# fugue-project/fugue

Hardware: NVIDIA H100
Metric: transform() rows/sec, hash-partitioned (num=256) identity map, 8-col table (higher is better)
Workload: dtype int64+f64 (byte moves; u64 hash arithmetic)

## Files before the change

### fugue_b200/csrc/fb_partition.cu

```cuda
#include <stdlib.h>

#include <mutex>

#include "fb_common.cuh"

namespace {

constexpr int kBlock = 512;
constexpr int kItems = 8;
constexpr int kTile = kBlock * kItems;
constexpr int kWarps = kBlock / 32;
constexpr int kCtasPerSm = 2;

struct FbCols {
  const void* src[FB_MAX_COLS];
  void* dst[FB_MAX_COLS];
  int32_t width[FB_MAX_COLS];
  int32_t ncols;
};

struct ChunkGeom {
  int64_t nrows;
  int64_t full_rows;
  int64_t tiles_per_chunk;
// ... 172 lines not shown
    const uint4 c = ((const uint4*)my)[lane];
    ((uint4*)(rec + kMetaCnt))[lane] = c;
    acc[0] += c.x & 0xFFFFu; acc[1] += c.x >> 16;
    acc[2] += c.y & 0xFFFFu; acc[3] += c.y >> 16;
    acc[4] += c.z & 0xFFFFu; acc[5] += c.z >> 16;
    acc[6] += c.w & 0xFFFFu; acc[7] += c.w >> 16;
    ((uint4*)my)[lane] = make_uint4(0, 0, 0, 0);
    __syncwarp();
  }
#pragma unroll
  for (int i = 0; i < 8; ++i)
    if (acc[i] != 0) atomicAdd(&s_hist[lane * 8 + i], acc[i]);
  __syncthreads();
  if (threadIdx.x < num) hist[(size_t)blockIdx.x * num + threadIdx.x] = s_hist[threadIdx.x];
}

__global__ void __launch_bounds__(256)
fb_scan_chunks_kernel(uint32_t* __restrict__ hist, uint32_t num, int32_t nchunks,
                      int64_t* __restrict__ totals) {
  __shared__ uint32_t s_warp[8];
  __shared__ uint32_t s_carry;
  const uint32_t b = blockIdx.x;
  const unsigned lane = threadIdx.x & 31, warp = threadIdx.x >> 5;
  if (threadIdx.x == 0) s_carry = 0;
  __syncthreads();
  for (int32_t c0 = 0; c0 < nchunks; c0 += 256) {
    int32_t c = c0 + threadIdx.x;
    uint32_t v = c < nchunks ? hist[(size_t)c * num + b] : 0;
    uint32_t x = v;
#pragma unroll
    for (int o = 1; o < 32; o <<= 1) {
      uint32_t y = __shfl_up_sync(0xFFFFFFFFu, x, o);
      if (lane >= (unsigned)o) x += y;
    }
    if (lane == 31) s_warp[warp] = x;
    __syncthreads();
    uint32_t wbase = 0;
    for (unsigned w = 0; w < warp; ++w) wbase += s_warp[w];
    uint32_t carry = s_carry;
    if (c < nchunks) hist[(size_t)c * num + b] = carry + wbase + x - v;
    __syncthreads();
    if (threadIdx.x == 255) s_carry = carry + wbase + x;
    __syncthreads();
  }
  if (threadIdx.x == 0) totals[b] = (int64_t)s_carry;
}

__global__ void __launch_bounds__(1024)
fb_scan_parts_kernel(int64_t* __restrict__ offsets, uint32_t num) {
  __shared__ int64_t s_warp[32];
  __shared__ int64_t s_carry;
  const unsigned lane = threadIdx.x & 31, warp = threadIdx.x >> 5;
  if (threadIdx.x == 0) s_carry = 0;
  __syncthreads();
  for (uint32_t b0 = 0; b0 < num; b0 += 1024) {
    uint32_t b = b0 + threadIdx.x;
    int64_t v = b < num ? offsets[b] : 0;
    int64_t x = v;
#pragma unroll
    for (int o = 1; o < 32; o <<= 1) {
      int64_t y = __shfl_up_sync(0xFFFFFFFFu, x, o);
      if (lane >= (unsigned)o) x += y;
    }
    if (lane == 31) s_warp[warp] = x;
    __syncthreads();
    int64_t wbase = 0;
    for (unsigned w = 0; w < warp; ++w) wbase += s_warp[w];
    int64_t carry = s_carry;
    if (b < num) offsets[b] = carry + wbase + x - v;
    __syncthreads();
    if (threadIdx.x == 1023) s_carry = carry + wbase + x;
    __syncthreads();
  }
  if (threadIdx.x == 0) offsets[num] = s_carry;
}

__host__ __device__ inline uint32_t nb_padded(uint32_t num) { return (num + 1 + 3) & ~3u; }

__host__ __device__ inline size_t scatter_smem_bytes(uint32_t num) {
  size_t nbp = nb_padded(num);
  return 2 * (size_t)kTile * 8 + (3 + (size_t)kWarps) * nbp * 4 + 32 * 4 + (size_t)kTile * 2;
}

constexpr int kMaxPer = (FB_MAX_PARTITIONS + 1 + kBlock - 1) / kBlock;

struct TileCtx {
  uint64_t* buf;
  uint32_t* delta;
  uint32_t* cursor;
  uint32_t* bin_start;
  uint32_t* cnt;
  uint32_t* scanw;
  uint16_t* pid_sorted;
  uint32_t nbp;
};

template <typename T, bool kFull>
__device__ __forceinline__ void load_col(const void* __restrict__ src, int64_t warp_row0, int warp_rows,
                                         unsigned lane, T (&v)[kItems]) {
  const T* __restrict__ p = (const T*)src + warp_row0 + lane;
#pragma unroll
  for (int r = 0; r < kItems; ++r)
    if (kFull || r * 32 + (int)lane < warp_rows) v[r] = __ldg(p + r * 32);
}

template <typename T, bool kFull>
__device__ __forceinline__ void move_columns(const FbCols& cols, const TileCtx& cx,
                                             const uint32_t (&pos)[kItems], const uint32_t (&dst)[kItems],
                                             int64_t warp_row0, int warp_rows, int tile_rows,
                                             unsigned lane, int& phase) {
  int c = 0;
  while (c < cols.ncols && cols.width[c] != (int)sizeof(T)) ++c;
  if (c >= cols.ncols) return;
  T v[kItems];
  load_col<T, kFull>(cols.src[c], warp_row0, warp_rows, lane, v);
  while (c < cols.ncols) {
    T* __restrict__ buf = (T*)(cx.buf + (size_t)(phase & 1) * kTile);
#pragma unroll
    for (int r = 0; r < kItems; ++r) buf[pos[r]] = v[r];
    int nxt = c + 1;
    while (nxt < cols.ncols && cols.width[nxt] != (int)sizeof(T)) ++nxt;
    if (nxt < cols.ncols) load_col<T, kFull>(cols.src[nxt], warp_row0, warp_rows, lane, v);
    __syncthreads();
    T* __restrict__ out = (T*)cols.dst[c];
#pragma unroll
    for (int k = 0; k < kItems; ++k) {
      const int j = k * kBlock + (int)threadIdx.x;
      if (kFull || j < tile_rows) out[dst[k]] = buf[j];
    }
    ++phase;
    c = nxt;
  }
}

template <bool kSingleU64, int kBits, bool kFull, bool kAll8>
__device__ __forceinline__ void scatter_tile(const FbKeys& keys, const FbDiv& dv, const uint32_t num,
                                             const FbCols& cols, const TileCtx& cx,
                                             const int64_t tile_row0, const int tile_rows, int& phase) {
  const unsigned lane = threadIdx.x & 31, warp = threadIdx.x >> 5;
  const unsigned lt = fb_lanemask_lt();
  const uint32_t nb = num + 1;
  const uint32_t nbp = cx.nbp;
  uint32_t* __restrict__ my_cnt = cx.cnt + warp * nbp;
  const int64_t warp_row0 = tile_row0 + (int64_t)warp * (32 * kItems);
  const int warp_rows = tile_rows - (int)warp * (32 * kItems);

  uint32_t pid[kItems];
#pragma unroll
  for (int r = 0; r < kItems; ++r) {
    const bool ok = kFull || (r * 32 + (int)lane) < warp_rows;
    pid[r] = ok ? compute_pid<kSingleU64>(keys, dv, warp_row0 + r * 32 + lane) : num;
  }

  uint32_t pos[kItems];
#pragma unroll
  for (int r = 0; r < kItems; ++r) {
    const unsigned m = match_lanes<kBits + (kFull ? 0 : 1)>(pid[r], 0xFFFFFFFFu);
    const unsigned before = __popc(m & lt);
    uint32_t old = 0;
    if (before == 0) {
      old = my_cnt[pid[r]];
      my_cnt[pid[r]] = old + __popc(m);
    }
    __syncwarp();
    old = __shfl_sync(0xFFFFFFFFu, old, __ffs(m) - 1);
    pos[r] = old + before;
  }
  __syncthreads();

  {
    const uint32_t per = (nb + kBlock - 1) / kBlock;
    const uint32_t b0 = threadIdx.x * per;
    uint32_t tot[kMaxPer];
    uint32_t sum = 0;
#pragma unroll
    for (int i = 0; i < kMaxPer; ++i) {
      tot[i] = 0;
      if ((uint32_t)i < per && b0 + i < nb) {
        uint32_t run = 0;
#pragma unroll
        for (int w = 0; w < kWarps; ++w) {
          const uint32_t t = cx.cnt[w * nbp + b0 + i];
          cx.cnt[w * nbp + b0 + i] = run;
          run += t;
        }
        tot[i] = run;
        sum += run;
      }
    }
    uint32_t x = sum;
#pragma unroll
    for (int o = 1; o < 32; o <<= 1) {
      const uint32_t y = __shfl_up_sync(0xFFFFFFFFu, x, o);
      if (lane >= (unsigned)o) x += y;
    }
    if (lane == 31) cx.scanw[warp] = x;
    __syncthreads();
    uint32_t run = x - sum;
    {
      const uint32_t wt = lane < kWarps ? cx.scanw[lane] : 0;
#pragma unroll
      for (int w = 0; w < kWarps; ++w) {
        const uint32_t v = __shfl_sync(0xFFFFFFFFu, wt, w);
        if ((unsigned)w < warp) run += v;
      }
    }
#pragma unroll
    for (int i = 0; i < kMaxPer; ++i) {
      if ((uint32_t)i < per && b0 + i < nb) {
        const uint32_t cur = cx.cursor[b0 + i];
        cx.bin_start[b0 + i] = run;
        cx.delta[b0 + i] = cur - run;
        cx.cursor[b0 + i] = cur + tot[i];
        run += tot[i];
      }
    }
  }
  __syncthreads();

#pragma unroll
  for (int r = 0; r < kItems; ++r) {
    pos[r] += cx.bin_start[pid[r]] + my_cnt[pid[r]];
    cx.pid_sorted[pos[r]] = (uint16_t)pid[r];
  }
  __syncthreads();
  uint32_t dst[kItems];
#pragma unroll
  for (int k = 0; k < kItems; ++k) {
    const int j = k * kBlock + (int)threadIdx.x;
    dst[k] = cx.delta[cx.pid_sorted[j]] + (uint32_t)j;
  }
  for (uint32_t i = threadIdx.x; i < (uint32_t)kWarps * nbp; i += kBlock) cx.cnt[i] = 0;

  move_columns<uint64_t, kFull>(cols, cx, pos, dst, warp_row0, warp_rows, tile_rows, lane, phase);
  if (!kAll8) {
    move_columns<uint32_t, kFull>(cols, cx, pos, dst, warp_row0, warp_rows, tile_rows, lane, phase);
    move_columns<uint16_t, kFull>(cols, cx, pos, dst, warp_row0, warp_rows, tile_rows, lane, phase);
    move_columns<uint8_t, kFull>(cols, cx, pos, dst, warp_row0, warp_rows, tile_rows, lane, phase);
  }
  __syncthreads();
}

template <bool kSingleU64, int kBits, bool kAll8>
__global__ void __launch_bounds__(kBlock, kCtasPerSm)
fb_scatter_kernel(FbKeys keys, FbDiv dv, uint32_t num, ChunkGeom g, int chunk0,
                  const uint32_t* __restrict__ chunk_base, const int64_t* __restrict__ part_offsets,
                  FbCols cols) {
  extern __shared__ __align__(128) uint64_t smem64[];
  TileCtx cx;
  cx.nbp = nb_padded(num);
  cx.buf = smem64;
  cx.delta = (uint32_t*)(smem64 + 2 * kTile);
  cx.cursor = cx.delta + cx.nbp;
  cx.bin_start = cx.cursor + cx.nbp;
  cx.cnt = cx.bin_start + cx.nbp;
  cx.scanw = cx.cnt + kWarps * cx.nbp;
  cx.pid_sorted = (uint16_t*)(cx.scanw + 32);

  const int chunk = chunk0 + (int)blockIdx.x;
  int64_t chunk_row0, chunk_row1;
  chunk_range(g, chunk, chunk_row0, chunk_row1);

  for (uint32_t b = threadIdx.x; b < cx.nbp; b += kBlock)
    cx.cursor[b] = b < num ? (uint32_t)part_offsets[b] + chunk_base[(size_t)chunk * num + b] : 0u;
  for (uint32_t i = threadIdx.x; i < (uint32_t)kWarps * cx.nbp; i += kBlock) cx.cnt[i] = 0;
  __syncthreads();

  int phase = 0;
  for (int64_t tile_row0 = chunk_row0; tile_row0 < chunk_row1; tile_row0 += kTile) {
    const int64_t left = chunk_row1 - tile_row0;
    if (left >= kTile)
      scatter_tile<kSingleU64, kBits, true, kAll8>(keys, dv, num, cols, cx, tile_row0, kTile, phase);
    else
      scatter_tile<kSingleU64, kBits, false, kAll8>(keys, dv, num, cols, cx, tile_row0, (int)left, phase);
  }
}

constexpr int kSwcMaxCols = 8;
constexpr uint32_t kSwcMaxNum = 256;

__device__ __forceinline__ uint32_t smem_u32(const void* p) { return (uint32_t)__cvta_generic_to_shared(p); }

__device__ __forceinline__ void mbar_init(uint32_t bar, uint32_t count) {
  asm volatile("mbarrier.init.shared::cta.b64 [%0], %1;" ::"r"(bar), "r"(count) : "memory");
}
__device__ __forceinline__ void mbar_expect_tx(uint32_t bar, uint32_t bytes) {
  asm volatile("mbarrier.arrive.expect_tx.shared::cta.b64 _, [%0], %1;" ::"r"(bar), "r"(bytes) : "memory");
}
__device__ __forceinline__ void mbar_arrive_relaxed(uint32_t bar) {
  asm volatile("mbarrier.arrive.relaxed.cta.shared::cta.b64 _, [%0];" ::"r"(bar) : "memory");
}
__device__ __forceinline__ void mbar_wait(uint32_t bar, uint32_t parity) {
  asm volatile(
      "{\n"
      ".reg .pred p;\n"
      "FB_WAIT:\n"
      "mbarrier.try_wait.parity.shared::cta.b64 p, [%0], %1;\n"
      "@p bra FB_DONE;\n"
      "bra FB_WAIT;\n"
      "FB_DONE:\n"
      "}\n" ::"r"(bar), "r"(parity)
      : "memory");
}
__device__ __forceinline__ uint64_t l2_policy_evict_first() {
  uint64_t pol;
  asm volatile("createpolicy.fractional.L2::evict_first.b64 %0, 1.0;" : "=l"(pol));
  return pol;
}
__device__ __forceinline__ uint64_t l2_policy_evict_last() {
  uint64_t pol;
  asm volatile("createpolicy.fractional.L2::evict_last.b64 %0, 1.0;" : "=l"(pol));
  return pol;
}
__device__ __forceinline__ void tma_load_1d(uint32_t dst_smem, const void* src, uint32_t bytes, uint32_t bar,
                                            uint64_t policy) {
  asm volatile(
      "cp.async.bulk.shared::cluster.global.mbarrier::complete_tx::bytes.L2::cache_hint [%0], [%1], %2, [%3], %4;"
      ::"r"(dst_smem), "l"(src), "r"(bytes), "r"(bar), "l"(policy)
      : "memory");
}

constexpr int kWsMoverWarps = 16, kWsRankWarps = 8;
constexpr int kWsMovers = kWsMoverWarps * 32, kWsRankers = kWsRankWarps * 32;
constexpr int kWsThreads = kWsMovers + kWsRankers + 128;
constexpr int kWsG = 16;
constexpr int kWsGWide = 4;
constexpr int kWsMinStages = 3;
constexpr int kWsRankItems = 16;
constexpr uint32_t kWsProducerRegs = 24, kWsRankerRegs = 64, kWsMoverRegs = 88;
static_assert(128 * kWsProducerRegs + kWsRankers * kWsRankerRegs + kWsMovers * kWsMoverRegs <= kWsThreads * 72,
              "setmaxnreg: the roles take more registers than the launch gives the CTA");
constexpr int kMoveBatch = 8;

struct WsUnits {
  const uint64_t* src[FB_MAX_COLS];
  uint64_t* dst[FB_MAX_COLS];
  int32_t nunits;
  int32_t per_group;
  int32_t ngroups;
};

struct WsMap {
  const uint64_t* src2[FB_MAX_COLS];
  uint64_t a[FB_MAX_COLS], b[FB_MAX_COLS], c[FB_MAX_COLS];
  int32_t mode[FB_MAX_COLS];
};

__device__ __forceinline__ uint64_t ws_apply_map(int mode, bool two, uint64_t x, uint64_t y, uint64_t a, uint64_t b,
                                                 uint64_t c) {
  if (mode == 1) {
    double r = __dmul_rn(__longlong_as_double((long long)a), __longlong_as_double((long long)x));
    if (two) r = __dadd_rn(r, __dmul_rn(__longlong_as_double((long long)b), __longlong_as_double((long long)y)));
    return (uint64_t)__double_as_longlong(__dadd_rn(r, __longlong_as_double((long long)c)));
  }
  if (mode == 2) return a * x + (two ? b * y : 0ULL) + c;
  return x;
}

template <int G, int RI>
__host__ __device__ inline size_t ws_book_bytes(uint32_t num, int ncols) {
  constexpr size_t kT = (size_t)kWsRankers * RI;
  const size_t nbp = nb_padded(num);
  const size_t E = (size_t)num * (G - 1);
  size_t b = 64 * 8;
  b += (size_t)ncols * E * 8;
  b += (kT + E) * 4;
  b += 5 * nbp * 4 + 64 * 4;
  b += ((E * 2 + 15) / 16) * 16;
  b += 2 * (size_t)kMetaBytes + 128;
  return b;
}

__device__ __forceinline__ void mbar_arrive(uint32_t bar) {
  asm volatile("mbarrier.arrive.shared::cta.b64 _, [%0];" ::"r"(bar) : "memory");
}
__device__ __forceinline__ void mover_sync() { asm volatile("bar.sync 1, %0;" ::"n"(kWsMovers) : "memory"); }
__device__ __forceinline__ void ranker_sync() { asm volatile("bar.sync 2, %0;" ::"n"(kWsRankers) : "memory"); }
template <uint32_t N>
__device__ __forceinline__ void setmaxnreg_dec() { asm volatile("setmaxnreg.dec.sync.aligned.u32 %0;" ::"n"(N)); }
template <uint32_t N>
__device__ __forceinline__ void setmaxnreg_inc() { asm volatile("setmaxnreg.inc.sync.aligned.u32 %0;" ::"n"(N)); }

template <int kBits, int G, int kWsRankItems, bool kMap>
__global__ void __launch_bounds__(kWsThreads, 1)
fb_scatter_ws_kernel(WsUnits units, uint32_t num, ChunkGeom g, int nstages,
                     const uint8_t* __restrict__ meta,
                     const uint32_t* __restrict__ chunk_base, const int64_t* __restrict__ part_offsets,
                     const __grid_constant__ WsMap map) {
  constexpr uint32_t T = (uint32_t)kWsRankers * kWsRankItems;
  static_assert(T == (uint32_t)kTile, "pass 1 ranks tiles of kTile rows");
  static_assert(G >= 2 && G <= 16 && (G & (G - 1)) == 0, "G must be a power of two <= 16");
  constexpr uint32_t GM = G - 1;
  constexpr uint32_t kStageBytes = T * 8;
  constexpr int kSlotRounds = ((int)T + (int)kSwcMaxNum * (G - 1) + kWsMovers - 1) / kWsMovers;
  constexpr int kEntryRoundsM = ((int)kSwcMaxNum * (G - 1) + kWsMovers - 1) / kWsMovers;
  extern __shared__ __align__(128) uint64_t smem64[];
  const uint32_t nbp = nb_padded(num);
  const uint32_t E = num * GM;
  const int grp = (int)blockIdx.x % units.ngroups;
  const int chunk_first = (int)blockIdx.x / units.ngroups, chunk_step = (int)gridDim.x / units.ngroups;
  const int u0 = grp * units.per_group;
  const int ncols = min(units.per_group, units.nunits - u0);
  uint64_t* ring = smem64;
  uint64_t* bars = ring + (size_t)nstages * T;
  uint64_t* carry = bars + 64;
  uint32_t* slotinfo = (uint32_t*)(carry + (size_t)ncols * E);
  uint32_t* wpos = slotinfo + T + E;
  uint32_t* kcnt = wpos + nbp;
  uint32_t* binfo = kcnt + nbp;
  uint32_t* wstart = binfo + nbp;
  uint32_t* wdelta = wstart + nbp;
  uint32_t* scanw = wdelta + nbp;
  uint16_t* carryinfo = (uint16_t*)(scanw + 64);
  uint8_t* metabuf = (uint8_t*)(((uintptr_t)(carryinfo + E) + 127) & ~(uintptr_t)127);

  const unsigned lane = threadIdx.x & 31, warp = threadIdx.x >> 5;
  const uint32_t bar_full = smem_u32(bars), bar_empty = smem_u32(bars + 16);
  const uint32_t bar_pid_full = smem_u32(bars + 32), bar_pid_empty = smem_u32(bars + 34);
  const uint32_t bar_slots_ready = smem_u32(bars + 36), bar_slots_free = smem_u32(bars + 37);
  const uint32_t bar_flush_done = smem_u32(bars + 38);

  if (threadIdx.x == 0) {
    for (int s = 0; s < nstages; ++s) {
      mbar_init(bar_full + 8 * s, 1);
      mbar_init(bar_empty + 8 * s, kWsMoverWarps);
    }
    for (int i = 0; i < 2; ++i) {
      mbar_init(bar_pid_full + 8 * i, 1);
      mbar_init(bar_pid_empty + 8 * i, kWsRankWarps);
    }
    mbar_init(bar_slots_ready, kWsRankWarps);
    mbar_init(bar_slots_free, kWsMoverWarps);
    mbar_init(bar_flush_done, kWsMoverWarps);
    asm volatile("fence.mbarrier_init.release.cluster;" ::: "memory");
  }
  __syncthreads();

  if (warp >= kWsMoverWarps + kWsRankWarps) {
    setmaxnreg_dec<kWsProducerRegs>();
    if (warp == kWsMoverWarps + kWsRankWarps && lane == 0) {
      const uint64_t pol = l2_policy_evict_first(), meta_pol = l2_policy_evict_last();
      const uint32_t ring_s = smem_u32(ring), meta_s = smem_u32(metabuf);
      uint32_t s = 0, ph = 0, seq = 0;
      int chunk = chunk_first;
      int64_t r0 = 0, r1 = 0, t0 = 0;
      bool have = chunk < g.nchunks_full;
      if (have) { chunk_range(g, chunk, r0, r1); t0 = r0; }
      auto load_pid = [&](int64_t row0, uint32_t q) {
        const uint32_t b = q & 1, pp = (q >> 1) & 1;
        mbar_wait(bar_pid_empty + 8 * b, pp ^ 1);
        mbar_expect_tx(bar_pid_full + 8 * b, kMetaBytes);
        tma_load_1d(meta_s + b * kMetaBytes, meta + (size_t)(row0 / T) * kMetaBytes, kMetaBytes,
                    bar_pid_full + 8 * b, meta_pol);
      };
      if (have) load_pid(t0, 0);
      while (have) {
        int nchunk = chunk;
        int64_t nr0 = r0, nr1 = r1, nt0 = t0 + T;
        bool nhave = true;
        if (nt0 >= r1) {
          nchunk = chunk + chunk_step;
          nhave = nchunk < g.nchunks_full;
          if (nhave) { chunk_range(g, nchunk, nr0, nr1); nt0 = nr0; }
        }
        if (nhave) load_pid(nt0, seq + 1);
        for (int u = u0; u < u0 + ncols; ++u) {
          mbar_wait(bar_empty + 8 * s, ph ^ 1);
          mbar_expect_tx(bar_full + 8 * s, kStageBytes);
          tma_load_1d(ring_s + s * kStageBytes, units.src[u] + t0, kStageBytes, bar_full + 8 * s, pol);
          if (++s == (uint32_t)nstages) { s = 0; ph ^= 1; }
          if constexpr (kMap) {
            if (map.src2[u] != nullptr) {
              mbar_wait(bar_empty + 8 * s, ph ^ 1);
              mbar_expect_tx(bar_full + 8 * s, kStageBytes);
              tma_load_1d(ring_s + s * kStageBytes, map.src2[u] + t0, kStageBytes, bar_full + 8 * s, pol);
              if (++s == (uint32_t)nstages) { s = 0; ph ^= 1; }
            }
          }
        }
        chunk = nchunk; r0 = nr0; r1 = nr1; t0 = nt0; have = nhave;
        ++seq;
      }
    }
    return;
  }

  if (warp >= kWsMoverWarps) {
    setmaxnreg_dec<kWsRankerRegs>();
    const unsigned rw = warp - kWsMoverWarps;
    const unsigned rtid = threadIdx.x - kWsMovers;
    uint32_t seq = 0, cseq = 0;
    for (int chunk = chunk_first; chunk < g.nchunks_full; chunk += chunk_step, ++cseq) {
      int64_t r0, r1;
      chunk_range(g, chunk, r0, r1);
      if (cseq > 0) mbar_wait(bar_flush_done, (cseq - 1) & 1);
      ranker_sync();
      for (uint32_t b = rtid; b < nbp; b += kWsRankers) {
        const uint32_t p0 = b < num ? (uint32_t)part_offsets[b] + chunk_base[(size_t)chunk * num + b] : 0u;
        wpos[b] = p0 & ~GM;
        kcnt[b] = (p0 & GM) | ((p0 & GM) << 8);
      }
      ranker_sync();
      for (int64_t t0 = r0; t0 < r1; t0 += T, ++seq) {
        const uint32_t pb = seq & 1, pph = (seq >> 1) & 1;
        mbar_wait(bar_pid_full + 8 * pb, pph);
        const uint8_t* __restrict__ rec = metabuf + pb * kMetaBytes;
        const uint32_t b = rtid;
        uint32_t n = 0, w = 0, kold = 0, phold = 0, wp_old = 0;
        if (b < num) n = ((const uint16_t*)(rec + kMetaCnt))[b];
        if (b < num) {
          const uint32_t kc = kcnt[b];
          kold = kc & 0xFFu;
          phold = kc >> 8;
          wp_old = wpos[b];
          const uint32_t end = wp_old + kold + n;
          const uint32_t aend = end & ~GM;
          if (aend > wp_old) {
            w = aend - wp_old;
            wpos[b] = aend;
            kcnt[b] = end - aend;
          } else {
            kcnt[b] = (kold + n) | (phold << 8);
          }
          binfo[b] = kold | (w << 8);
        }
        uint32_t xw = w;
#pragma unroll
        for (int o = 1; o < 32; o <<= 1) {
          const uint32_t yw = __shfl_up_sync(0xFFFFFFFFu, xw, o);
          if (lane >= (unsigned)o) xw += yw;
        }
        if (lane == 31) scanw[8 + rw] = xw;
        ranker_sync();
        uint32_t bw = xw - w;
        {
          const uint32_t tw = lane < kWsRankWarps ? scanw[8 + lane] : 0;
#pragma unroll
          for (int wi = 0; wi < kWsRankWarps; ++wi) {
            const uint32_t vw = __shfl_sync(0xFFFFFFFFu, tw, wi);
            if ((unsigned)wi < rw) bw += vw;
          }
        }
        if (seq > 0) mbar_wait(bar_slots_free, (seq - 1) & 1);
        if (b < num) {
          wstart[b] = bw;
          wdelta[b] = wp_old - bw;
        }
        if (rtid == kWsRankers - 1) scanw[40] = bw + w;
        ranker_sync();
#pragma unroll
        for (int r = 0; r < kWsRankItems; ++r) {
          const uint32_t row = r * kWsRankers + rtid;
          const uint32_t pb2 = rec[row];
          const uint32_t bi = binfo[pb2];
          const uint32_t i = (bi & 0xFFu) + ((const uint16_t*)(rec + kMetaRank))[row];
          const uint32_t ww = bi >> 8;
          if (i < ww) slotinfo[wstart[pb2] + i] = (pb2 << 16) | row;
          else carryinfo[pb2 * GM + (i - ww)] = (uint16_t)row;
        }
        __syncwarp();
        if (lane == 0) mbar_arrive_relaxed(bar_pid_empty + 8 * pb);
        if (b < num) {
#pragma unroll
          for (uint32_t i = 0; i < GM; ++i) {
            const uint32_t e = b * GM + i;
            const uint32_t desc = i < phold ? 0xFFFFu : T + e;
            if (i < kold) {
              if (i < w) slotinfo[bw + i] = (b << 16) | desc;
              else carryinfo[e] = (uint16_t)desc;
            }
            if (w + i >= kold + n) carryinfo[e] = 0xFFFFu;
          }
        }
        ranker_sync();
        if (lane == 0) mbar_arrive(bar_slots_ready);
      }
    }
    return;
  }

  setmaxnreg_inc<kWsMoverRegs>();
  uint32_t s = 0, ph = 0, seq = 0;
  for (int chunk = chunk_first; chunk < g.nchunks_full; chunk += chunk_step) {
    int64_t r0, r1;
    chunk_range(g, chunk, r0, r1);
    for (int64_t t0 = r0; t0 < r1; t0 += T, ++seq) {
      mbar_wait(bar_slots_ready, seq & 1);
      const uint32_t W = scanw[40];
      uint32_t srcd[kSlotRounds], dst[kSlotRounds];
#pragma unroll
      for (int k = 0; k < kSlotRounds; ++k) {
        const uint32_t j = k * kWsMovers + threadIdx.x;
        srcd[k] = 0xFFFFu;
        dst[k] = 0;
        if (j < W) {
          const uint32_t info = slotinfo[j];
          srcd[k] = info & 0xFFFFu;
          dst[k] = wdelta[info >> 16] + j;
        }
      }
      uint32_t csrc[kEntryRoundsM];
#pragma unroll
      for (int q = 0; q < kEntryRoundsM; ++q) {
        const uint32_t e = q * kWsMovers + threadIdx.x;
        const uint32_t d = e < E ? (uint32_t)carryinfo[e] : 0xFFFFu;
        csrc[q] = d < T ? d : 0xFFFFu;
      }
      __syncwarp();
      if (lane == 0) mbar_arrive(bar_slots_free);

      for (int u = 0; u < ncols; ++u) {
        mbar_wait(bar_full + 8 * s, ph);
        const uint64_t* __restrict__ st = ring + (size_t)s * T;
        uint64_t* __restrict__ out = units.dst[u0 + u];
        uint64_t* __restrict__ cbuf = carry + (size_t)u * E;
        uint32_t s2 = s;
        bool two = false;
        const uint64_t* __restrict__ st2 = st;
        int mode = 0;
        uint64_t ma = 0, mb = 0, mc = 0;
        if constexpr (kMap) {
          mode = map.mode[u0 + u];
          two = map.src2[u0 + u] != nullptr;
          if (two) {
            s2 = s + 1 == (uint32_t)nstages ? 0 : s + 1;
            mbar_wait(bar_full + 8 * s2, s2 == 0 ? ph ^ 1 : ph);
            st2 = ring + (size_t)s2 * T;
          }
          ma = map.a[u0 + u]; mb = map.b[u0 + u]; mc = map.c[u0 + u];
        }
        auto staged = [&](uint32_t r) -> uint64_t {
          if constexpr (kMap) return ws_apply_map(mode, two, st[r], st2[r], ma, mb, mc);
          else return st[r];
        };
#pragma unroll
        for (int k0 = 0; k0 < kSlotRounds; k0 += kMoveBatch) {
          uint64_t v[kMoveBatch];
#pragma unroll
          for (int k = 0; k < kMoveBatch; ++k)
            if (k0 + k < kSlotRounds && srcd[k0 + k] != 0xFFFFu)
              v[k] = srcd[k0 + k] < T ? staged(srcd[k0 + k]) : cbuf[srcd[k0 + k] - T];
#pragma unroll
          for (int k = 0; k < kMoveBatch; ++k)
            if (k0 + k < kSlotRounds && srcd[k0 + k] != 0xFFFFu) out[dst[k0 + k]] = v[k];
        }
        mover_sync();
#pragma unroll
        for (int q = 0; q < kEntryRoundsM; ++q)
          if (csrc[q] != 0xFFFFu) cbuf[q * kWsMovers + threadIdx.x] = staged(csrc[q]);
        __syncwarp();
        if (lane == 0) {
          mbar_arrive_relaxed(bar_empty + 8 * s);
          if (kMap && two) mbar_arrive_relaxed(bar_empty + 8 * s2);
        }
        if (++s == (uint32_t)nstages) { s = 0; ph ^= 1; }
        if (kMap && two) {
          if (++s == (uint32_t)nstages) { s = 0; ph ^= 1; }
        }
      }
      if (ncols == 1) mover_sync();
    }
    mover_sync();
    for (int u = 0; u < ncols; ++u) {
      uint64_t* __restrict__ out = units.dst[u0 + u];
      const uint64_t* __restrict__ cbuf = carry + (size_t)u * E;
#pragma unroll
      for (int q = 0; q < kEntryRoundsM; ++q) {
        const uint32_t e = q * kWsMovers + threadIdx.x;
        if (e < E) {
          const uint32_t b = e / GM, i = e - b * GM;
          const uint32_t kc = kcnt[b];
          if (i < (kc & 0xFFu) && i >= (kc >> 8)) out[wpos[b] + i] = cbuf[e];
        }
      }
    }
    __syncwarp();
    if (lane == 0) mbar_arrive(bar_flush_done);
  }
}

__global__ void fb_bits_to_bytes_kernel(const uint8_t* __restrict__ bits, int64_t bit_offset,
                                        int64_t nrows, uint8_t* __restrict__ out) {
  int64_t i = (int64_t)blockIdx.x * blockDim.x + threadIdx.x;
  int64_t stride = (int64_t)gridDim.x * blockDim.x;
  for (; i < nrows; i += stride) {
    int64_t j = i + bit_offset;
    out[i] = (bits[j >> 3] >> (j & 7)) & 1;
  }
}

__global__ void fb_bytes_to_bits_kernel(const uint8_t* __restrict__ bytes, int64_t nrows,
                                        uint8_t* __restrict__ out, unsigned long long* null_count) {
  int64_t nbytes = (nrows + 7) >> 3;
  int64_t i = (int64_t)blockIdx.x * blockDim.x + threadIdx.x;
  int64_t stride = (int64_t)gridDim.x * blockDim.x;
  unsigned long long nulls = 0;
  for (; i < nbytes; i += stride) {
    uint8_t v = 0;
#pragma unroll
    for (int k = 0; k < 8; ++k) {
      int64_t r = i * 8 + k;
      if (r < nrows) {
        if (bytes[r]) v |= (uint8_t)(1u << k);
        else ++nulls;
      }
    }
    out[i] = v;
  }
  if (null_count != nullptr && nulls) atomicAdd(null_count, nulls);
}

inline int bits_for(uint32_t num) { return num <= 16 ? 4 : (num <= 256 ? 8 : 10); }

#define FB_DISPATCH_SB(single, bits, LAUNCH)                 \
  do {                                                       \
    if (single) {                                            \
      if (bits == 4) LAUNCH(true, 4);                        \
      else if (bits == 8) LAUNCH(true, 8);                   \
      else LAUNCH(true, 10);                                 \
    } else {                                                 \
      if (bits == 4) LAUNCH(false, 4);                       \
      else if (bits == 8) LAUNCH(false, 8);                  \
      else LAUNCH(false, 10);                                \
    }                                                        \
  } while (0)

template <typename K>
cudaError_t optin(K kernel, size_t bytes) {
  return cudaFuncSetAttribute(kernel, cudaFuncAttributeMaxDynamicSharedMemorySize, (int)bytes);
}

cudaError_t ensure_smem_optin(int dev) {
  static std::mutex mu;
  static uint64_t done = 0;
  std::lock_guard<std::mutex> lock(mu);
  if (dev >= 0 && dev < 64 && (done >> dev) & 1) return cudaSuccess;
  const size_t sc = scatter_smem_bytes(FB_MAX_PARTITIONS);
  const size_t hs = (size_t)kHistWarps * FB_MAX_PARTITIONS * sizeof(uint32_t);
  cudaError_t e = cudaSuccess;
#define FB_OPTIN(S, B)                                                   \
  do {                                                                   \
    if (e == cudaSuccess) e = optin(fb_scatter_kernel<S, B, true>, sc);  \
    if (e == cudaSuccess) e = optin(fb_scatter_kernel<S, B, false>, sc); \
    if (e == cudaSuccess) e = optin(fb_hist_kernel<S, B>, hs);           \
  } while (0)
  {
    int smem_max = 0;
    if (e == cudaSuccess) e = cudaDeviceGetAttribute(&smem_max, cudaDevAttrMaxSharedMemoryPerBlockOptin, dev);
#define FB_OPTIN_WS(G)                                                                                        \
  do {                                                                                                        \
    if (e == cudaSuccess) e = optin(fb_scatter_ws_kernel<4, G, kWsRankItems, false>, (size_t)smem_max);       \
    if (e == cudaSuccess) e = optin(fb_scatter_ws_kernel<8, G, kWsRankItems, false>, (size_t)smem_max);       \
    if (e == cudaSuccess) e = optin(fb_scatter_ws_kernel<4, G, kWsRankItems, true>, (size_t)smem_max);        \
    if (e == cudaSuccess) e = optin(fb_scatter_ws_kernel<8, G, kWsRankItems, true>, (size_t)smem_max);        \
  } while (0)
    FB_OPTIN_WS(kWsG);
    FB_OPTIN_WS(kWsGWide);
#undef FB_OPTIN_WS
  }
  FB_OPTIN(true, 4); FB_OPTIN(true, 8); FB_OPTIN(true, 10);
  FB_OPTIN(false, 4); FB_OPTIN(false, 8); FB_OPTIN(false, 10);
#undef FB_OPTIN
  if (e == cudaSuccess && dev >= 0 && dev < 64) done |= (1ull << dev);
  return e;
}

bool single_u64_key(int nkeys, const int32_t* widths, const uint8_t* const* valid) {
  return nkeys == 1 && widths[0] == 8 && (valid == nullptr || valid[0] == nullptr);
}

int fill_keys(FbKeys& k, int nkeys, const void* const* ptrs, const int32_t* widths,
              const uint8_t* const* valid) {
  FB_CHECK(nkeys >= 1 && nkeys <= FB_MAX_KEYS, "nkeys=%d out of range [1,%d]", nkeys, FB_MAX_KEYS);
  memset(&k, 0, sizeof(k));
  k.nkeys = nkeys;
  k.digit_shift = -1;
  for (int i = 0; i < nkeys; ++i) {
    FB_CHECK(widths[i] == 1 || widths[i] == 2 || widths[i] == 4 || widths[i] == 8,
             "key %d has unsupported width %d", i, widths[i]);
    FB_CHECK(ptrs[i] != nullptr, "key %d pointer is NULL", i);
    k.ptr[i] = ptrs[i];
    k.width[i] = widths[i];
    k.valid[i] = valid ? valid[i] : nullptr;
  }
  return 0;
}

struct PlanLayout {
  size_t hist_bytes;
  size_t pid_offset;
  size_t total_bytes;
};

PlanLayout plan_layout(const ChunkGeom& g, uint32_t num) {
  PlanLayout l;
  l.hist_bytes = (((size_t)g.nchunks * num * sizeof(uint32_t)) + 255) & ~(size_t)255;
  l.pid_offset = l.hist_bytes + 256;
  l.total_bytes = l.pid_offset + (num <= kSwcMaxNum ? (size_t)(g.full_rows / kTile) * kMetaBytes : 0) + 256;
  return l;
}

}

extern "C" {

size_t fb_partition_scratch_bytes(int dev, int64_t nrows, uint32_t num_partitions) {
  if (nrows < 0 || num_partitions == 0) return 0;
  ChunkGeom g = make_geom(dev, nrows);
  return plan_layout(g, num_partitions).total_bytes;
}

int fb_partition_ids(int dev, void* stream, int64_t nrows, int nkeys, const void* const* key_ptrs,
                     const int32_t* key_widths, const uint8_t* const* key_valid,
                     uint32_t num_partitions, uint32_t* out_pids) {
  FB_CHECK(nrows >= 0, "nrows < 0");
  FB_CHECK(num_partitions >= 1, "num_partitions must be >= 1");
  if (nrows == 0) return 0;
  FbDeviceGuard guard(dev);
  FB_CHECK(guard.ok, "cannot select device %d", dev);
  FbKeys k;
  if (int rc = fill_keys(k, nkeys, key_ptrs, key_widths, key_valid)) return rc;
  FbDiv dv = fb_make_div(num_partitions);
  int64_t blocks = (nrows + 255) / 256;
  int64_t maxb = (int64_t)fb_sm_count(dev) * 16;
  if (blocks > maxb) blocks = maxb;
  cudaStream_t st = (cudaStream_t)stream;
  if (single_u64_key(nkeys, key_widths, key_valid))
    fb_pid_kernel<true><<<(unsigned)blocks, 256, 0, st>>>(k, dv, nrows, out_pids);
  else
    fb_pid_kernel<false><<<(unsigned)blocks, 256, 0, st>>>(k, dv, nrows, out_pids);
  FB_CUDA(cudaGetLastError());
  return 0;
}

int fb_row_hash64(int dev, void* stream, int64_t nrows, int nkeys, const void* const* key_ptrs,
                  const int32_t* key_widths, const uint8_t* const* key_valid, uint64_t* out_hash) {
  FB_CHECK(nrows >= 0, "nrows < 0");
  if (nrows == 0) return 0;
  FbDeviceGuard guard(dev);
  FB_CHECK(guard.ok, "cannot select device %d", dev);
  FbKeys k;
  if (int rc = fill_keys(k, nkeys, key_ptrs, key_widths, key_valid)) return rc;
  int64_t blocks = (nrows + 255) / 256;
  int64_t maxb = (int64_t)fb_sm_count(dev) * 16;
  if (blocks > maxb) blocks = maxb;
  fb_row_hash_kernel<<<(unsigned)blocks, 256, 0, (cudaStream_t)stream>>>(k, nrows, out_hash);
  FB_CUDA(cudaGetLastError());
  return 0;
}

static int plan_impl(int dev, void* stream, int64_t nrows, const FbKeys& k, bool single,
                     uint32_t num_partitions, void* scratch, size_t scratch_bytes,
                     int64_t* out_part_offsets) {
  FB_CHECK(nrows >= 0, "nrows < 0");
  FB_CHECK(nrows < ((int64_t)1 << 32), "nrows=%lld exceeds the 2^32-1 rows one call handles",
           (long long)nrows);
  FB_CHECK(num_partitions >= 1 && num_partitions <= FB_MAX_PARTITIONS,
           "num_partitions=%u out of range [1,%d]", num_partitions, FB_MAX_PARTITIONS);
  FB_CHECK(out_part_offsets != nullptr, "out_part_offsets is NULL");
  FbDeviceGuard guard(dev);
  FB_CHECK(guard.ok, "cannot select device %d", dev);
  cudaStream_t st = (cudaStream_t)stream;
  if (nrows == 0) {
    FB_CUDA(cudaMemsetAsync(out_part_offsets, 0, sizeof(int64_t) * ((size_t)num_partitions + 1), st));
    return 0;
  }
  ChunkGeom g = make_geom(dev, nrows);
  PlanLayout l = plan_layout(g, num_partitions);
  FB_CHECK(scratch != nullptr && scratch_bytes >= l.total_bytes,
           "scratch too small: need %zu bytes, got %zu", l.total_bytes, scratch_bytes);
  FbDiv dv = fb_make_div(num_partitions);
  uint32_t* hist = (uint32_t*)scratch;
  size_t smem = (size_t)kHistWarps * num_partitions * sizeof(uint32_t);
  FB_CUDA(ensure_smem_optin(dev));
  const int bits = bits_for(num_partitions);
  int hist_chunk0 = 0;
  if (num_partitions <= kSwcMaxNum && g.nchunks_full > 0) {
    uint8_t* meta = (uint8_t*)scratch + l.pid_offset;
#define FB_LAUNCH_RANK(S, B, STAGED) \
  fb_rank_tile_kernel<S, B, STAGED><<<g.nchunks_full, kRankBlock, 0, st>>>(k, dv, num_partitions, g, hist, meta)
    if (single) {
      if (bits == 4) FB_LAUNCH_RANK(true, 4, true);
      else FB_LAUNCH_RANK(true, 8, true);
    } else if (k.digit_shift >= 0) {
      if (bits == 4) FB_LAUNCH_RANK(false, 4, true);
      else FB_LAUNCH_RANK(false, 8, true);
    } else {
      if (bits == 4) FB_LAUNCH_RANK(false, 4, false);
      else FB_LAUNCH_RANK(false, 8, false);
    }
#undef FB_LAUNCH_RANK
    FB_CUDA(cudaGetLastError());
    hist_chunk0 = g.nchunks_full;
  }
  if (hist_chunk0 < g.nchunks) {
#define FB_LAUNCH_HIST(S, B)                                                                       \
  fb_hist_kernel<S, B><<<g.nchunks - hist_chunk0, kHistBlock, smem, st>>>(k, dv, num_partitions, g, \
                                                                          hist_chunk0, hist)
    FB_DISPATCH_SB(single, bits, FB_LAUNCH_HIST);
#undef FB_LAUNCH_HIST
    FB_CUDA(cudaGetLastError());
  }
  fb_scan_chunks_kernel<<<num_partitions, 256, 0, st>>>(hist, num_partitions, g.nchunks, out_part_offsets);
  FB_CUDA(cudaGetLastError());
  fb_scan_parts_kernel<<<1, 1024, 0, st>>>(out_part_offsets, num_partitions);
  FB_CUDA(cudaGetLastError());
  return 0;
}

int fb_partition_plan(int dev, void* stream, int64_t nrows, int nkeys, const void* const* key_ptrs,
                      const int32_t* key_widths, const uint8_t* const* key_valid,
                      uint32_t num_partitions, void* scratch, size_t scratch_bytes,
                      int64_t* out_part_offsets) {
  FbKeys k;
  if (nrows == 0) {
    memset(&k, 0, sizeof(k));
    k.nkeys = 1;
    k.digit_shift = -1;
    return plan_impl(dev, stream, 0, k, false, num_partitions, scratch, scratch_bytes, out_part_offsets);
  }
  if (int rc = fill_keys(k, nkeys, key_ptrs, key_widths, key_valid)) return rc;
  return plan_impl(dev, stream, nrows, k, single_u64_key(nkeys, key_widths, key_valid), num_partitions,
                   scratch, scratch_bytes, out_part_offsets);
}

__global__ void fb_map_tail_kernel(int ncols, const void* const* __restrict__ x_ptrs, const fb_map_unit* __restrict__ maps,
                                   int64_t row0, int64_t nrows, uint64_t* __restrict__ tmp) {
  const int64_t n = nrows - row0;
  for (int64_t i = (int64_t)blockIdx.x * blockDim.x + threadIdx.x; i < n * ncols; i += (int64_t)gridDim.x * blockDim.x) {
    const int c = (int)(i / n);
    const int64_t r = row0 + i % n;
    const fb_map_unit m = maps[c];
    const uint64_t x = ((const uint64_t*)x_ptrs[c])[r];
    const uint64_t y = m.src2 != nullptr ? ((const uint64_t*)m.src2)[r] : 0;
    tmp[(size_t)c * kTile + (size_t)(i % n)] = ws_apply_map(m.mode, m.src2 != nullptr, x, y, m.a, m.b, m.c);
  }
}

static int apply_impl(int dev, void* stream, int64_t nrows, const FbKeys& k, bool single,
                      uint32_t num_partitions, const void* scratch, size_t scratch_bytes,
                      const int64_t* part_offsets, int ncols, const void* const* col_ptrs,
                      const int32_t* col_widths, void* const* out_col_ptrs, int sm_reserve = 0,
                      const fb_map_unit* maps = nullptr, void* tail_tmp = nullptr, int cols_per_launch_req = 0) {
  FB_CHECK(nrows >= 0 && nrows < ((int64_t)1 << 32), "nrows out of range");
  FB_CHECK(num_partitions >= 1 && num_partitions <= FB_MAX_PARTITIONS,
           "num_partitions=%u out of range [1,%d]", num_partitions, FB_MAX_PARTITIONS);
  FB_CHECK(ncols >= 0, "ncols < 0");
  if (nrows == 0 || ncols == 0) return 0;
  FbDeviceGuard guard(dev);
  FB_CHECK(guard.ok, "cannot select device %d", dev);
  ChunkGeom g = make_geom(dev, nrows);
  PlanLayout l = plan_layout(g, num_partitions);
  FB_CHECK(scratch != nullptr && scratch_bytes >= l.total_bytes, "scratch too small");
  FbDiv dv = fb_make_div(num_partitions);
  cudaStream_t st = (cudaStream_t)stream;
  const size_t smem = scatter_smem_bytes(num_partitions);
  FB_CUDA(ensure_smem_optin(dev));
  const int bits = bits_for(num_partitions);

  for (int c = 0; c < ncols; ++c) {
    const int w = col_widths[c];
    FB_CHECK(w == 1 || w == 2 || w == 4 || w == 8, "column %d has unsupported width %d", c, w);
    FB_CHECK(col_ptrs[c] != nullptr && out_col_ptrs[c] != nullptr, "column %d pointer is NULL", c);
  }

  const void* const* gen_src = col_ptrs;
  auto launch_generic = [&](const int* idx, int n, int chunk0, int nch) -> int {
    for (int c0 = 0; c0 < n && nch > 0; c0 += FB_MAX_COLS) {
      FbCols cols;
      memset(&cols, 0, sizeof(cols));
      cols.ncols = n - c0 < FB_MAX_COLS ? n - c0 : FB_MAX_COLS;
      bool all8 = true;
      for (int c = 0; c < cols.ncols; ++c) {
        cols.src[c] = gen_src[idx[c0 + c]];
        cols.dst[c] = out_col_ptrs[idx[c0 + c]];
        cols.width[c] = col_widths[idx[c0 + c]];
        all8 = all8 && cols.width[c] == 8;
      }
#define FB_LAUNCH_SCATTER(S, B)                                                                        \
  do {                                                                                                 \
// ... 239 lines not shown
```

Measured before the change: 18.00 billion.

## Assign each CTA one contiguous run of chunks and drop per-chunk flush barrier

Each warp-specialized scatter CTA now processes a contiguous range of chunks, computed by ws_chunk_run, instead of a strided set of chunks. Per-partition write positions are initialised once and carried across chunk boundaries. This removes the per-chunk carry flush and the flush_done barrier that stalled the rankers between chunks. The TMA load policy for staged column data also changes from L2 evict_first to evict_normal. The change relies on chunk_base for consecutive chunks being consistent with carrying state across them, and the L2 policy change may affect cache behaviour.

```diff
diff --git a/fugue_b200/csrc/fb_partition.cu b/fugue_b200/csrc/fb_partition.cu
--- a/fugue_b200/csrc/fb_partition.cu
+++ b/fugue_b200/csrc/fb_partition.cu
@@ -498,9 +498,9 @@
       "}\n" ::"r"(bar), "r"(parity)
       : "memory");
 }
-__device__ __forceinline__ uint64_t l2_policy_evict_first() {
+__device__ __forceinline__ uint64_t l2_policy_evict_normal() {
   uint64_t pol;
-  asm volatile("createpolicy.fractional.L2::evict_first.b64 %0, 1.0;" : "=l"(pol));
+  asm volatile("createpolicy.fractional.L2::evict_normal.b64 %0, 1.0;" : "=l"(pol));
   return pol;
 }
 __device__ __forceinline__ uint64_t l2_policy_evict_last() {
@@ -535,6 +535,14 @@
   int32_t per_group;
   int32_t ngroups;
 };
+
+__device__ __forceinline__ void ws_chunk_run(const ChunkGeom& g, int i, int S, int& c0, int64_t& r0, int64_t& r1) {
+  c0 = (int)((int64_t)i * g.nchunks_full / S);
+  const int c1 = (int)((int64_t)(i + 1) * g.nchunks_full / S);
+  int64_t unused;
+  chunk_range(g, c0, r0, unused);
+  chunk_range(g, c1 - 1, unused, r1);
+}
 
 struct WsMap {
   const uint64_t* src2[FB_MAX_COLS];
@@ -594,7 +602,9 @@
   const uint32_t nbp = nb_padded(num);
   const uint32_t E = num * GM;
   const int grp = (int)blockIdx.x % units.ngroups;
-  const int chunk_first = (int)blockIdx.x / units.ngroups, chunk_step = (int)gridDim.x / units.ngroups;
+  int chunk0;
+  int64_t row0, row1;
+  ws_chunk_run(g, (int)blockIdx.x / units.ngroups, (int)gridDim.x / units.ngroups, chunk0, row0, row1);
   const int u0 = grp * units.per_group;
   const int ncols = min(units.per_group, units.nunits - u0);
   uint64_t* ring = smem64;
@@ -614,7 +624,6 @@
   const uint32_t bar_full = smem_u32(bars), bar_empty = smem_u32(bars + 16);
   const uint32_t bar_pid_full = smem_u32(bars + 32), bar_pid_empty = smem_u32(bars + 34);
   const uint32_t bar_slots_ready = smem_u32(bars + 36), bar_slots_free = smem_u32(bars + 37);
-  const uint32_t bar_flush_done = smem_u32(bars + 38);
 
   if (threadIdx.x == 0) {
     for (int s = 0; s < nstages; ++s) {
@@ -627,7 +636,6 @@
     }
     mbar_init(bar_slots_ready, kWsRankWarps);
     mbar_init(bar_slots_free, kWsMoverWarps);
-    mbar_init(bar_flush_done, kWsMoverWarps);
     asm volatile("fence.mbarrier_init.release.cluster;" ::: "memory");
   }
   __syncthreads();
@@ -635,31 +643,19 @@
   if (warp >= kWsMoverWarps + kWsRankWarps) {
     setmaxnreg_dec<kWsProducerRegs>();
     if (warp == kWsMoverWarps + kWsRankWarps && lane == 0) {
-      const uint64_t pol = l2_policy_evict_first(), meta_pol = l2_policy_evict_last();
+      const uint64_t pol = l2_policy_evict_normal(), meta_pol = l2_policy_evict_last();
       const uint32_t ring_s = smem_u32(ring), meta_s = smem_u32(metabuf);
       uint32_t s = 0, ph = 0, seq = 0;
-      int chunk = chunk_first;
-      int64_t r0 = 0, r1 = 0, t0 = 0;
-      bool have = chunk < g.nchunks_full;
-      if (have) { chunk_range(g, chunk, r0, r1); t0 = r0; }
-      auto load_pid = [&](int64_t row0, uint32_t q) {
+      auto load_pid = [&](int64_t t, uint32_t q) {
         const uint32_t b = q & 1, pp = (q >> 1) & 1;
         mbar_wait(bar_pid_empty + 8 * b, pp ^ 1);
         mbar_expect_tx(bar_pid_full + 8 * b, kMetaBytes);
-        tma_load_1d(meta_s + b * kMetaBytes, meta + (size_t)(row0 / T) * kMetaBytes, kMetaBytes,
+        tma_load_1d(meta_s + b * kMetaBytes, meta + (size_t)(t / T) * kMetaBytes, kMetaBytes,
                     bar_pid_full + 8 * b, meta_pol);
       };
-      if (have) load_pid(t0, 0);
-      while (have) {
-        int nchunk = chunk;
-        int64_t nr0 = r0, nr1 = r1, nt0 = t0 + T;
-        bool nhave = true;
-        if (nt0 >= r1) {
-          nchunk = chunk + chunk_step;
-          nhave = nchunk < g.nchunks_full;
-          if (nhave) { chunk_range(g, nchunk, nr0, nr1); nt0 = nr0; }
-        }
-        if (nhave) load_pid(nt0, seq + 1);
+      load_pid(row0, 0);
+      for (int64_t t0 = row0; t0 < row1; t0 += T, ++seq) {
+        if (t0 + T < row1) load_pid(t0 + T, seq + 1);
         for (int u = u0; u < u0 + ncols; ++u) {
           mbar_wait(bar_empty + 8 * s, ph ^ 1);
           mbar_expect_tx(bar_full + 8 * s, kStageBytes);
@@ -674,8 +670,6 @@
             }
           }
         }
-        chunk = nchunk; r0 = nr0; r1 = nr1; t0 = nt0; have = nhave;
-        ++seq;
       }
     }
     return;
@@ -685,193 +679,181 @@
     setmaxnreg_dec<kWsRankerRegs>();
     const unsigned rw = warp - kWsMoverWarps;
     const unsigned rtid = threadIdx.x - kWsMovers;
-    uint32_t seq = 0, cseq = 0;
-    for (int chunk = chunk_first; chunk < g.nchunks_full; chunk += chunk_step, ++cseq) {
-      int64_t r0, r1;
-      chunk_range(g, chunk, r0, r1);
-      if (cseq > 0) mbar_wait(bar_flush_done, (cseq - 1) & 1);
+    for (uint32_t b = rtid; b < nbp; b += kWsRankers) {
+      const uint32_t p0 = b < num ? (uint32_t)part_offsets[b] + chunk_base[(size_t)chunk0 * num + b] : 0u;
+      wpos[b] = p0 & ~GM;
+      kcnt[b] = (p0 & GM) | ((p0 & GM) << 8);
+    }
+    ranker_sync();
+    uint32_t seq = 0;
+    for (int64_t t0 = row0; t0 < row1; t0 += T, ++seq) {
+      const uint32_t pb = seq & 1, pph = (seq >> 1) & 1;
+      mbar_wait(bar_pid_full + 8 * pb, pph);
+      const uint8_t* __restrict__ rec = metabuf + pb * kMetaBytes;
+      const uint32_t b = rtid;
+      uint32_t n = 0, w = 0, kold = 0, phold = 0, wp_old = 0;
+      if (b < num) n = ((const uint16_t*)(rec + kMetaCnt))[b];
+      if (b < num) {
+        const uint32_t kc = kcnt[b];
+        kold = kc & 0xFFu;
+        phold = kc >> 8;
+        wp_old = wpos[b];
+        const uint32_t end = wp_old + kold + n;
+        const uint32_t aend = end & ~GM;
+        if (aend > wp_old) {
+          w = aend - wp_old;
+          wpos[b] = aend;
+          kcnt[b] = end - aend;
+        } else {
+          kcnt[b] = (kold + n) | (phold << 8);
+        }
+        binfo[b] = kold | (w << 8);
+      }
+      uint32_t xw = w;
+#pragma unroll
+      for (int o = 1; o < 32; o <<= 1) {
+        const uint32_t yw = __shfl_up_sync(0xFFFFFFFFu, xw, o);
+        if (lane >= (unsigned)o) xw += yw;
+      }
+      if (lane == 31) scanw[8 + rw] = xw;
       ranker_sync();
-      for (uint32_t b = rtid; b < nbp; b += kWsRankers) {
-        const uint32_t p0 = b < num ? (uint32_t)part_offsets[b] + chunk_base[(size_t)chunk * num + b] : 0u;
-        wpos[b] = p0 & ~GM;
-        kcnt[b] = (p0 & GM) | ((p0 & GM) << 8);
-      }
+      uint32_t bw = xw - w;
+      {
+        const uint32_t tw = lane < kWsRankWarps ? scanw[8 + lane] : 0;
+#pragma unroll
+        for (int wi = 0; wi < kWsRankWarps; ++wi) {
+          const uint32_t vw = __shfl_sync(0xFFFFFFFFu, tw, wi);
+          if ((unsigned)wi < rw) bw += vw;
+        }
+      }
+      if (seq > 0) mbar_wait(bar_slots_free, (seq - 1) & 1);
+      if (b < num) {
+        wstart[b] = bw;
+        wdelta[b] = wp_old - bw;
+      }
+      if (rtid == kWsRankers - 1) scanw[40] = bw + w;
       ranker_sync();
-      for (int64_t t0 = r0; t0 < r1; t0 += T, ++seq) {
-        const uint32_t pb = seq & 1, pph = (seq >> 1) & 1;
-        mbar_wait(bar_pid_full + 8 * pb, pph);
-        const uint8_t* __restrict__ rec = metabuf + pb * kMetaBytes;
-        const uint32_t b = rtid;
-        uint32_t n = 0, w = 0, kold = 0, phold = 0, wp_old = 0;
-        if (b < num) n = ((const uint16_t*)(rec + kMetaCnt))[b];
-        if (b < num) {
-          const uint32_t kc = kcnt[b];
-          kold = kc & 0xFFu;
-          phold = kc >> 8;
-          wp_old = wpos[b];
-          const uint32_t end = wp_old + kold + n;
-          const uint32_t aend = end & ~GM;
-          if (aend > wp_old) {
-            w = aend - wp_old;
-            wpos[b] = aend;
-            kcnt[b] = end - aend;
-          } else {
-            kcnt[b] = (kold + n) | (phold << 8);
+#pragma unroll
+      for (int r = 0; r < kWsRankItems; ++r) {
+        const uint32_t row = r * kWsRankers + rtid;
+        const uint32_t pb2 = rec[row];
+        const uint32_t bi = binfo[pb2];
+        const uint32_t i = (bi & 0xFFu) + ((const uint16_t*)(rec + kMetaRank))[row];
+        const uint32_t ww = bi >> 8;
+        if (i < ww) slotinfo[wstart[pb2] + i] = (pb2 << 16) | row;
+        else carryinfo[pb2 * GM + (i - ww)] = (uint16_t)row;
+      }
+      __syncwarp();
+      if (lane == 0) mbar_arrive_relaxed(bar_pid_empty + 8 * pb);
+      if (b < num) {
+#pragma unroll
+        for (uint32_t i = 0; i < GM; ++i) {
+          const uint32_t e = b * GM + i;
+          const uint32_t desc = i < phold ? 0xFFFFu : T + e;
+          if (i < kold) {
+            if (i < w) slotinfo[bw + i] = (b << 16) | desc;
+            else carryinfo[e] = (uint16_t)desc;
           }
-          binfo[b] = kold | (w << 8);
+          if (w + i >= kold + n) carryinfo[e] = 0xFFFFu;
         }
-        uint32_t xw = w;
-#pragma unroll
-        for (int o = 1; o < 32; o <<= 1) {
-          const uint32_t yw = __shfl_up_sync(0xFFFFFFFFu, xw, o);
-          if (lane >= (unsigned)o) xw += yw;
-        }
-        if (lane == 31) scanw[8 + rw] = xw;
-        ranker_sync();
-        uint32_t bw = xw - w;
-        {
-          const uint32_t tw = lane < kWsRankWarps ? scanw[8 + lane] : 0;
-#pragma unroll
-          for (int wi = 0; wi < kWsRankWarps; ++wi) {
-            const uint32_t vw = __shfl_sync(0xFFFFFFFFu, tw, wi);
-            if ((unsigned)wi < rw) bw += vw;
-          }
-        }
-        if (seq > 0) mbar_wait(bar_slots_free, (seq - 1) & 1);
-        if (b < num) {
-          wstart[b] = bw;
-          wdelta[b] = wp_old - bw;
-        }
-        if (rtid == kWsRankers - 1) scanw[40] = bw + w;
-        ranker_sync();
-#pragma unroll
-        for (int r = 0; r < kWsRankItems; ++r) {
-          const uint32_t row = r * kWsRankers + rtid;
-          const uint32_t pb2 = rec[row];
-          const uint32_t bi = binfo[pb2];
-          const uint32_t i = (bi & 0xFFu) + ((const uint16_t*)(rec + kMetaRank))[row];
-          const uint32_t ww = bi >> 8;
-          if (i < ww) slotinfo[wstart[pb2] + i] = (pb2 << 16) | row;
-          else carryinfo[pb2 * GM + (i - ww)] = (uint16_t)row;
-        }
-        __syncwarp();
-        if (lane == 0) mbar_arrive_relaxed(bar_pid_empty + 8 * pb);
-        if (b < num) {
-#pragma unroll
-          for (uint32_t i = 0; i < GM; ++i) {
-            const uint32_t e = b * GM + i;
-            const uint32_t desc = i < phold ? 0xFFFFu : T + e;
-            if (i < kold) {
-              if (i < w) slotinfo[bw + i] = (b << 16) | desc;
-              else carryinfo[e] = (uint16_t)desc;
-            }
-            if (w + i >= kold + n) carryinfo[e] = 0xFFFFu;
-          }
-        }
-        ranker_sync();
-        if (lane == 0) mbar_arrive(bar_slots_ready);
-      }
+      }
+      ranker_sync();
+      if (lane == 0) mbar_arrive(bar_slots_ready);
     }
     return;
   }
 
   setmaxnreg_inc<kWsMoverRegs>();
   uint32_t s = 0, ph = 0, seq = 0;
-  for (int chunk = chunk_first; chunk < g.nchunks_full; chunk += chunk_step) {
-    int64_t r0, r1;
-    chunk_range(g, chunk, r0, r1);
-    for (int64_t t0 = r0; t0 < r1; t0 += T, ++seq) {
-      mbar_wait(bar_slots_ready, seq & 1);
-      const uint32_t W = scanw[40];
-      uint32_t srcd[kSlotRounds], dst[kSlotRounds];
-#pragma unroll
-      for (int k = 0; k < kSlotRounds; ++k) {
-        const uint32_t j = k * kWsMovers + threadIdx.x;
-        srcd[k] = 0xFFFFu;
-        dst[k] = 0;
-        if (j < W) {
-          const uint32_t info = slotinfo[j];
-          srcd[k] = info & 0xFFFFu;
-          dst[k] = wdelta[info >> 16] + j;
+  for (int64_t t0 = row0; t0 < row1; t0 += T, ++seq) {
+    mbar_wait(bar_slots_ready, seq & 1);
+    const uint32_t W = scanw[40];
+    uint32_t srcd[kSlotRounds], dst[kSlotRounds];
+#pragma unroll
+    for (int k = 0; k < kSlotRounds; ++k) {
+      const uint32_t j = k * kWsMovers + threadIdx.x;
+      srcd[k] = 0xFFFFu;
+      dst[k] = 0;
+      if (j < W) {
+        const uint32_t info = slotinfo[j];
+        srcd[k] = info & 0xFFFFu;
+        dst[k] = wdelta[info >> 16] + j;
+      }
+    }
+    uint32_t csrc[kEntryRoundsM];
+#pragma unroll
+    for (int q = 0; q < kEntryRoundsM; ++q) {
+      const uint32_t e = q * kWsMovers + threadIdx.x;
+      const uint32_t d = e < E ? (uint32_t)carryinfo[e] : 0xFFFFu;
+      csrc[q] = d < T ? d : 0xFFFFu;
+    }
+    __syncwarp();
+    if (lane == 0) mbar_arrive(bar_slots_free);
+
+    for (int u = 0; u < ncols; ++u) {
+      mbar_wait(bar_full + 8 * s, ph);
+      const uint64_t* __restrict__ st = ring + (size_t)s * T;
+      uint64_t* __restrict__ out = units.dst[u0 + u];
+      uint64_t* __restrict__ cbuf = carry + (size_t)u * E;
+      uint32_t s2 = s;
+      bool two = false;
+      const uint64_t* __restrict__ st2 = st;
+      int mode = 0;
+      uint64_t ma = 0, mb = 0, mc = 0;
+      if constexpr (kMap) {
+        mode = map.mode[u0 + u];
+        two = map.src2[u0 + u] != nullptr;
+        if (two) {
+          s2 = s + 1 == (uint32_t)nstages ? 0 : s + 1;
+          mbar_wait(bar_full + 8 * s2, s2 == 0 ? ph ^ 1 : ph);
+          st2 = ring + (size_t)s2 * T;
         }
-      }
-      uint32_t csrc[kEntryRoundsM];
-#pragma unroll
-      for (int q = 0; q < kEntryRoundsM; ++q) {
-        const uint32_t e = q * kWsMovers + threadIdx.x;
-        const uint32_t d = e < E ? (uint32_t)carryinfo[e] : 0xFFFFu;
-        csrc[q] = d < T ? d : 0xFFFFu;
-      }
+        ma = map.a[u0 + u]; mb = map.b[u0 + u]; mc = map.c[u0 + u];
+      }
+      auto staged = [&](uint32_t r) -> uint64_t {
+        if constexpr (kMap) return ws_apply_map(mode, two, st[r], st2[r], ma, mb, mc);
+        else return st[r];
+      };
+#pragma unroll
+      for (int k0 = 0; k0 < kSlotRounds; k0 += kMoveBatch) {
+        uint64_t v[kMoveBatch];
+#pragma unroll
+        for (int k = 0; k < kMoveBatch; ++k)
+          if (k0 + k < kSlotRounds && srcd[k0 + k] != 0xFFFFu)
+            v[k] = srcd[k0 + k] < T ? staged(srcd[k0 + k]) : cbuf[srcd[k0 + k] - T];
+#pragma unroll
+        for (int k = 0; k < kMoveBatch; ++k)
+          if (k0 + k < kSlotRounds && srcd[k0 + k] != 0xFFFFu) out[dst[k0 + k]] = v[k];
+      }
+      mover_sync();
+#pragma unroll
+      for (int q = 0; q < kEntryRoundsM; ++q)
+        if (csrc[q] != 0xFFFFu) cbuf[q * kWsMovers + threadIdx.x] = staged(csrc[q]);
       __syncwarp();
-      if (lane == 0) mbar_arrive(bar_slots_free);
-
-      for (int u = 0; u < ncols; ++u) {
-        mbar_wait(bar_full + 8 * s, ph);
-        const uint64_t* __restrict__ st = ring + (size_t)s * T;
-        uint64_t* __restrict__ out = units.dst[u0 + u];
-        uint64_t* __restrict__ cbuf = carry + (size_t)u * E;
-        uint32_t s2 = s;
-        bool two = false;
-        const uint64_t* __restrict__ st2 = st;
-        int mode = 0;
-        uint64_t ma = 0, mb = 0, mc = 0;
-        if constexpr (kMap) {
-          mode = map.mode[u0 + u];
-          two = map.src2[u0 + u] != nullptr;
-          if (two) {
-            s2 = s + 1 == (uint32_t)nstages ? 0 : s + 1;
-            mbar_wait(bar_full + 8 * s2, s2 == 0 ? ph ^ 1 : ph);
-            st2 = ring + (size_t)s2 * T;
-          }
-          ma = map.a[u0 + u]; mb = map.b[u0 + u]; mc = map.c[u0 + u];
-        }
-        auto staged = [&](uint32_t r) -> uint64_t {
-          if constexpr (kMap) return ws_apply_map(mode, two, st[r], st2[r], ma, mb, mc);
-          else return st[r];
-        };
-#pragma unroll
-        for (int k0 = 0; k0 < kSlotRounds; k0 += kMoveBatch) {
-          uint64_t v[kMoveBatch];
-#pragma unroll
-          for (int k = 0; k < kMoveBatch; ++k)
-            if (k0 + k < kSlotRounds && srcd[k0 + k] != 0xFFFFu)
-              v[k] = srcd[k0 + k] < T ? staged(srcd[k0 + k]) : cbuf[srcd[k0 + k] - T];
-#pragma unroll
-          for (int k = 0; k < kMoveBatch; ++k)
-            if (k0 + k < kSlotRounds && srcd[k0 + k] != 0xFFFFu) out[dst[k0 + k]] = v[k];
-        }
-        mover_sync();
-#pragma unroll
-        for (int q = 0; q < kEntryRoundsM; ++q)
-          if (csrc[q] != 0xFFFFu) cbuf[q * kWsMovers + threadIdx.x] = staged(csrc[q]);
-        __syncwarp();
-        if (lane == 0) {
-          mbar_arrive_relaxed(bar_empty + 8 * s);
-          if (kMap && two) mbar_arrive_relaxed(bar_empty + 8 * s2);
-        }
+      if (lane == 0) {
+        mbar_arrive_relaxed(bar_empty + 8 * s);
+        if (kMap && two) mbar_arrive_relaxed(bar_empty + 8 * s2);
+      }
+      if (++s == (uint32_t)nstages) { s = 0; ph ^= 1; }
+      if (kMap && two) {
         if (++s == (uint32_t)nstages) { s = 0; ph ^= 1; }
-        if (kMap && two) {
-          if (++s == (uint32_t)nstages) { s = 0; ph ^= 1; }
-        }
-      }
-      if (ncols == 1) mover_sync();
-    }
-    mover_sync();
-    for (int u = 0; u < ncols; ++u) {
-      uint64_t* __restrict__ out = units.dst[u0 + u];
-      const uint64_t* __restrict__ cbuf = carry + (size_t)u * E;
-#pragma unroll
-      for (int q = 0; q < kEntryRoundsM; ++q) {
-        const uint32_t e = q * kWsMovers + threadIdx.x;
-        if (e < E) {
-          const uint32_t b = e / GM, i = e - b * GM;
-          const uint32_t kc = kcnt[b];
-          if (i < (kc & 0xFFu) && i >= (kc >> 8)) out[wpos[b] + i] = cbuf[e];
-        }
-      }
-    }
-    __syncwarp();
-    if (lane == 0) mbar_arrive(bar_flush_done);
+      }
+    }
+    if (ncols == 1) mover_sync();
+  }
+  mover_sync();
+  for (int u = 0; u < ncols; ++u) {
+    uint64_t* __restrict__ out = units.dst[u0 + u];
+    const uint64_t* __restrict__ cbuf = carry + (size_t)u * E;
+#pragma unroll
+    for (int q = 0; q < kEntryRoundsM; ++q) {
+      const uint32_t e = q * kWsMovers + threadIdx.x;
+      if (e < E) {
+        const uint32_t b = e / GM, i = e - b * GM;
+        const uint32_t kc = kcnt[b];
+        if (i < (kc & 0xFFu) && i >= (kc >> 8)) out[wpos[b] + i] = cbuf[e];
+      }
+    }
   }
 }
 
```

New measurement: 18.58 billion (median of 6 runs). 3.2% higher.
